# WeeFav/Visual-Odometry-GPU

Measured on AMD Instinct MI355X. Metric: ORB detect+describe frames/sec (1241x376, 8 lvls), higher is better.
Workload: dtype u8; 1 GPU; KITTI-shaped 1241x376 u8, 8 levels s=1.2, 1000 features, FAST-9 t=20, NMS 3x3, Harris top-N, blur5 all levels, BRIEF-256; batch=1024 frames/step/GPU resident in HBM (stream A); distinct_resident_batches=2, fast_early_exit=True, pyramid_blur_fused=True, pyramid_top_rows_first=True, pipelined_batches=True

## Files before the change

### visual-odometry-gpu_amd/csrc/orbx_kernels.hip

```cpp
#include <hip/hip_runtime.h>

#include <cstdlib>

#include "orbx_internal.h"
#include "orbx_math.h"
#include "orbx_wave.h"

__constant__ __attribute__((aligned(16))) int8_t c_pattern[1024] = {
#include "pattern_31.inc"
};


typedef uint16_t __attribute__((aligned(1))) u16_unaligned;

__device__ __forceinline__ void decode_tile(const OrbxTileMap& tm, int nlevels, int& l, int& tx, int& ty) {
  const int t = blockIdx.x;
  l = 0;
#pragma unroll 1
  for (int i = 1; i < nlevels; i++)
    if (t >= tm.begin[i]) l = i;
  const int local = t - tm.begin[l];
  ty = local / tm.tiles_x[l];
  tx = local - ty * tm.tiles_x[l];
}
// ... 6 lines not shown
}

typedef uint32_t __attribute__((aligned(1))) u32_unaligned;
struct __attribute__((packed, aligned(1))) uint2_unaligned {
  uint32_t x, y;
  __device__ operator uint2() const { return make_uint2(x, y); }
};

template <int ROWS, bool WIN8>
__device__ __forceinline__ void pyr_rows(const uint8_t* __restrict__ src, int in_stride, int w0, int h0,
                                         const OrbxResizeTap* __restrict__ ytaps, int yb, int lh,
                                         const uint32_t (&ofs)[4], const uint32_t (&cc)[4],
                                         __amdgpu_buffer_rsrc_t rout, uint32_t voff_st, uint32_t vmask, int pitch) {
  constexpr int NW = WIN8 ? 2 : 4;
  uint32_t q0[ROWS][NW], q1[ROWS][NW];
  int b0[ROWS], b1[ROWS];
  uint32_t sel[4];
  uint32_t base = 0;
  if (WIN8) {
    base = min(ofs[0], (uint32_t)(w0 - 8));
#pragma unroll
    for (int k = 0; k < 4; k++) {
      const uint32_t sb = ofs[k] - base;
      sel[k] = 0x0c000c00u | ((sb + 1) << 16) | sb;
    }
  }
#pragma unroll
  for (int r = 0; r < ROWS; r++) {
    const int y = min(yb + r, lh - 1);
    const OrbxResizeTap ty_ = ytaps[y];
    const int sy0 = min(max(ty_.ofs, 0), h0 - 1), sy1 = min(max(ty_.ofs + 1, 0), h0 - 1);
    const uint8_t* S0 = src + (size_t)sy0 * in_stride;
    const uint8_t* S1 = src + (size_t)sy1 * in_stride;
    b0[r] = ty_.c0;
    b1[r] = ty_.c1;
    if (WIN8) {
      const uint2 a = *reinterpret_cast<const uint2_unaligned*>(S0 + base);
      const uint2 b = *reinterpret_cast<const uint2_unaligned*>(S1 + base);
      q0[r][0] = a.x;
      q0[r][1] = a.y;
      q1[r][0] = b.x;
      q1[r][1] = b.y;
    } else {
#pragma unroll
      for (int k = 0; k < 4; k++) {
        q0[r][k] = *reinterpret_cast<const u16_unaligned*>(S0 + ofs[k]);
        q1[r][k] = *reinterpret_cast<const u16_unaligned*>(S1 + ofs[k]);
      }
    }
  }
#pragma unroll
  for (int r = 0; r < ROWS; r++) {
    uint32_t out = 0;
    const uint32_t bs0 = ((uint32_t)b0[r] << 12) & 0xffffffu, bs1 = ((uint32_t)b1[r] << 12) & 0xffffffu;
#pragma unroll
    for (int k = 0; k < 4; k++) {
      uint32_t p0, p1;
      if (WIN8) {
        p0 = __builtin_amdgcn_perm(q0[r][1], q0[r][0], sel[k]);
        p1 = __builtin_amdgcn_perm(q1[r][1], q1[r][0], sel[k]);
      } else {
        p0 = __builtin_amdgcn_perm(q0[r][k], q0[r][k], 0x0c010c00u);
        p1 = __builtin_amdgcn_perm(q1[r][k], q1[r][k], 0x0c010c00u);
      }
      const us2_t cw = __builtin_bit_cast(us2_t, cc[k]);
      const uint32_t r0 = __builtin_amdgcn_udot2(__builtin_bit_cast(us2_t, p0), cw, 0u, false);
      const uint32_t r1 = __builtin_amdgcn_udot2(__builtin_bit_cast(us2_t, p1), cw, 0u, false);
      const uint32_t t0 = (uint32_t)(((u64)(r0 & 0xfffff0u) * (u64)bs0) >> 32);
      const uint32_t t1 = (uint32_t)(((u64)(r1 & 0xfffff0u) * (u64)bs1) >> 32);
      out |= ((t0 + t1 + 2u) >> 2) << (8 * k);
    }
    const int y = yb + r;
    if (y < lh) __builtin_amdgcn_raw_buffer_store_b32(out & vmask, rout, voff_st, y * pitch, 0);
  }
}

__global__ __launch_bounds__(256) void k_pyramid2(const OrbxTileDesc* __restrict__ tiles, int n_tiles, int frame_bytes, int w0,
                                                  int h0, const uint8_t* __restrict__ in, int in_stride,
                                                  size_t in_frame_stride, const OrbxResizeTap* __restrict__ taps,
                                                  uint8_t* __restrict__ pyr) {
  if ((int)blockIdx.x >= n_tiles) return;
  const OrbxTileDesc d = tiles[blockIdx.x];
  struct {
    int w, h, pitch, xtab_off, ytab_off, win8;
  } L = {d.w, d.h, d.pitch, d.u0, d.u1, d.u2};
  const int l = d.l, tx = d.tx, ty = d.ty;
  const int rpw = d.f;
  const int f = blockIdx.y;
  const int lane = threadIdx.x & 63;
  const int wave = __builtin_amdgcn_readfirstlane(threadIdx.x >> 6);
  const uint8_t* src = in + (size_t)f * in_frame_stride;
  const int x = tx * 256 + lane * 4;
  const int yb = (ty * 4 + wave) * rpw;
  if (yb >= L.h) return;
  const int pitch = L.pitch, w = L.w;
  const __amdgpu_buffer_rsrc_t rout =
      __builtin_amdgcn_make_buffer_rsrc(pyr + (size_t)f * frame_bytes + d.img_off, 0, pitch * L.h, 0x00020000);
  const uint32_t voff_st = x < pitch ? (uint32_t)x : 0xffffffffu;
  const int nvalid = w - x;
  const uint32_t vmask = nvalid >= 4 ? 0xffffffffu : nvalid <= 0 ? 0u : ((1u << (8 * nvalid)) - 1u);

  if (l == 0) {
#pragma unroll
    for (int r = 0; r < 8; r++) {
      const int y = yb + r;
      if (r < rpw && y < L.h) {
        const uint8_t* row = src + (size_t)y * in_stride;
        uint32_t v = 0;
        if (nvalid >= 4 || (nvalid > 0 && y + 1 < L.h)) {
          v = *reinterpret_cast<const u32_unaligned*>(row + x);
        } else if (nvalid > 0) {
          for (int k = 0; k < nvalid; k++) v |= (uint32_t)row[x + k] << (8 * k);
        }
        __builtin_amdgcn_raw_buffer_store_b32(v & vmask, rout, voff_st, y * pitch, 0);
      }
    }
    return;
  }

  uint32_t ofs[4] = {0, 0, 0, 0}, cc[4] = {0, 0, 0, 0};
  if (nvalid > 0) {
    const uint4* tp = reinterpret_cast<const uint4*>(taps + L.xtab_off + x);
    const uint4 t01 = tp[0], t23 = tp[1];
    ofs[0] = t01.x; ofs[1] = t01.z; ofs[2] = t23.x; ofs[3] = t23.z;
    cc[0] = t01.y; cc[1] = t01.w; cc[2] = t23.y; cc[3] = t23.w;
  }
  const OrbxResizeTap* ytaps = taps + L.ytab_off;
  if (L.win8) {
    if (rpw == 8)
      pyr_rows<8, true>(src, in_stride, w0, h0, ytaps, yb, L.h, ofs, cc, rout, voff_st, vmask, pitch);
    else
      pyr_rows<4, true>(src, in_stride, w0, h0, ytaps, yb, L.h, ofs, cc, rout, voff_st, vmask, pitch);
  } else {
    pyr_rows<4, false>(src, in_stride, w0, h0, ytaps, yb, L.h, ofs, cc, rout, voff_st, vmask, pitch);
  }
}

#define BLUR_SROWS (ORBX_BLUR_TH + 4)
#define BLUR_SPITCH 72

__device__ __forceinline__ void blur_load_tile(uint8_t* s_src, const uint8_t* img, const OrbxLevel& L, int x0,
                                               int y0) {
  uint32_t* s32 = reinterpret_cast<uint32_t*>(s_src);
  for (int i = threadIdx.x; i < BLUR_SROWS * (BLUR_SPITCH / 4); i += 256) {
    const int row = i / (BLUR_SPITCH / 4), c = i - row * (BLUR_SPITCH / 4);
    const int gy = reflect101(y0 - 2 + row, L.h);
    const int gx = x0 - 4 + 4 * c;
    uint32_t v = 0;
    if (gx >= 0 && gx + 4 <= L.pitch) v = *reinterpret_cast<const uint32_t*>(img + (size_t)gy * L.pitch + gx);
    s32[i] = v;
  }
  __syncthreads();
  if (threadIdx.x < BLUR_SROWS) {
    uint8_t* row = s_src + threadIdx.x * BLUR_SPITCH;
    if (x0 == 0) {
      row[3] = row[5];
      row[2] = row[6];
    }
    const int rem = L.w - x0;
    if (rem <= ORBX_BLUR_TW + 1) {
#pragma unroll
      for (int k = 0; k < 2; k++) {
        const int x = L.w + k;
        const int col = x - x0 + 4;
        if (col < BLUR_SPITCH) row[col] = row[(2 * L.w - x - 2) - x0 + 4];
      }
    }
  }
  __syncthreads();
}

__global__ __launch_bounds__(256) void k_blur(OrbxPlan plan, OrbxTileMap tm, const uint8_t* __restrict__ src,
                                              uint8_t* __restrict__ dst, int first_level, int kind) {
  __shared__ __attribute__((aligned(16))) uint8_t s_src[BLUR_SROWS * BLUR_SPITCH];
  __shared__ __attribute__((aligned(16))) uint16_t s_h[BLUR_SROWS * ORBX_BLUR_TW];
  int l, tx, ty;
  decode_tile(tm, plan.nlevels, l, tx, ty);
  const OrbxLevel& L = plan.L[l];
  const int f = blockIdx.y;
  const uint8_t* img = src + (size_t)f * plan.frame_bytes + L.img_off;
  uint8_t* out = dst + (size_t)f * plan.frame_bytes + L.img_off;
  const int x0 = tx * ORBX_BLUR_TW, y0 = ty * ORBX_BLUR_TH;
  const int c4 = (threadIdx.x & 15) * 4, r = threadIdx.x >> 4;
  const int gy = y0 + r, gx = x0 + c4;

  if (l < first_level) {
    if (gy < L.h && gx < L.pitch)
      *reinterpret_cast<uint32_t*>(out + (size_t)gy * L.pitch + gx) =
          *reinterpret_cast<const uint32_t*>(img + (size_t)gy * L.pitch + gx);
    return;
  }
  blur_load_tile(s_src, img, L, x0, y0);

  uint32_t packed = 0;
  if (kind == 0) {
    for (int i = threadIdx.x; i < BLUR_SROWS * ORBX_BLUR_TW; i += 256) {
      const int row = i >> 6, c = i & 63;
      const uint8_t* p = s_src + row * BLUR_SPITCH + c + 2;
      s_h[i] = (uint16_t)(p[0] + 4 * p[1] + 6 * p[2] + 4 * p[3] + p[4]);
    }
    __syncthreads();
#pragma unroll
    for (int k = 0; k < 4; k++) {
      const uint16_t* h = s_h + r * ORBX_BLUR_TW + c4 + k;
      const uint32_t S = h[0] + 4u * h[ORBX_BLUR_TW] + 6u * h[2 * ORBX_BLUR_TW] + 4u * h[3 * ORBX_BLUR_TW] +
                         h[4 * ORBX_BLUR_TW];
      const uint32_t v = (S + 127u + ((S >> 8) & 1u)) >> 8;
      if (gx + k < L.w) packed |= v << (8 * k);
    }
  } else {
    const int kw[25] = {1, 4, 7, 4, 1, 4, 16, 26, 16, 4, 7, 26, 41, 26, 7, 4, 16, 26, 16, 4, 1, 4, 7, 4, 1};
#pragma unroll
    for (int k = 0; k < 4; k++) {
      uint32_t S = 0;
#pragma unroll
      for (int i = 0; i < 5; i++)
#pragma unroll
        for (int j = 0; j < 5; j++) S += (uint32_t)kw[i * 5 + j] * s_src[(r + i) * BLUR_SPITCH + c4 + k + 2 + j];
      const uint32_t v = (2u * S + 273u) / 546u;
      if (gx + k < L.w) packed |= v << (8 * k);
    }
  }
  if (gy < L.h && gx < L.pitch) *reinterpret_cast<uint32_t*>(out + (size_t)gy * L.pitch + gx) = packed;
}



__global__ __launch_bounds__(256) void k_compact(OrbxPlan plan, const u64* __restrict__ mask,
                                                 orbx_keypoint* __restrict__ cand,
                                                 int32_t* __restrict__ cand_count,
                                                 int32_t* __restrict__ cand_total, int need_total) {
  __shared__ int s_wsum[4];
  const int l = blockIdx.x, f = blockIdx.y;
  const OrbxLevel& L = plan.L[l];
  const u64* m = mask + (size_t)f * plan.mask_words + L.mask_off;
  orbx_keypoint* out = cand + (size_t)f * plan.cand_total + L.cand_off;
  const int nwords = L.h * L.mask_wpr;
  const int tid = threadIdx.x, lane = tid & 63, wave = tid >> 6;
  int base = 0;
  for (int w0 = 0; w0 < nwords; w0 += 256) {
    const int i = w0 + tid;
    u64 v = i < nwords ? m[i] : 0ull;
    const int c = __popcll(v);
    const int incl = wave_scan_incl(c);
    if (lane == 63) s_wsum[wave] = incl;
    __syncthreads();
    int woff = 0, tot = 0;
#pragma unroll
    for (int k = 0; k < 4; k++) {
      const int s = s_wsum[k];
      if (k < wave) woff += s;
      tot += s;
    }
    int pos = base + woff + incl - c;
    if (c && pos < L.cap) {
      const int y = i / L.mask_wpr, xw = i - y * L.mask_wpr;
      while (v && pos < L.cap) {
        const int b = __ffsll((long long)v) - 1;
        v &= v - 1;
        orbx_keypoint kp;
        kp.x = orbx_mask_x(L, xw, b);
        kp.y = y;
        out[pos++] = kp;
      }
    }
    base += tot;
    __syncthreads();
    if (!need_total && base >= L.cap) break;
  }
  if (tid == 0) {
    cand_total[f * plan.nlevels + l] = base;
    cand_count[f * plan.nlevels + l] = base < L.cap ? base : L.cap;
  }
}

__device__ __forceinline__ float harris_at(const uint8_t* img, int w, int h, int pitch, int x, int y,
                                           const float* __restrict__ g, int K, float kk) {
  const int r = K / 2;
  float a = 0.f, b = 0.f, c = 0.f;
  for (int i = 0; i < K; i++) {
    const int yy = reflect101(y - r + i, h);
    const uint8_t* r0 = img + (size_t)reflect101(yy - 1, h) * pitch;
    const uint8_t* r1 = img + (size_t)yy * pitch;
    const uint8_t* r2 = img + (size_t)reflect101(yy + 1, h) * pitch;
    for (int j = 0; j < K; j++) {
      const int xx = reflect101(x - r + j, w);
      const int xl = reflect101(xx - 1, w), xr = reflect101(xx + 1, w);
      const int p00 = r0[xl], p01 = r0[xx], p02 = r0[xr];
      const int p10 = r1[xl], p12 = r1[xr];
      const int p20 = r2[xl], p21 = r2[xx], p22 = r2[xr];
      const float gx = (float)((p02 + 2 * p12 + p22) - (p00 + 2 * p10 + p20));
      const float gy = (float)((p20 + 2 * p21 + p22) - (p00 + 2 * p01 + p02));
      const float wgt = g[i * K + j];
      a = __fadd_rn(a, __fmul_rn(__fmul_rn(gx, gx), wgt));
      c = __fadd_rn(c, __fmul_rn(__fmul_rn(gy, gy), wgt));
      b = __fadd_rn(b, __fmul_rn(__fmul_rn(gx, gy), wgt));
    }
  }
  const float det = __fsub_rn(__fmul_rn(a, c), __fmul_rn(b, b));
  const float trace = __fadd_rn(a, c);
  return __fsub_rn(det, __fmul_rn(__fmul_rn(kk, trace), trace));
}

template <int K>
__device__ __forceinline__ float harris_fast(const uint8_t* img, int w, int h, int pitch, int x, int y,
                                             const float* __restrict__ g, float kk) {
  constexpr int r = K / 2, P = K + 2;
  static_assert(P <= 9, "the third dword of a row supplies pixel 8 only");
  const int xs = x - r - 1;
  const int a0 = xs & ~3, off = xs - a0;
  const uint32_t sel_l = xs < 0 ? 0x03020102u : 0x03020100u;
  const uint32_t sel_r = xs + P - 1 >= w ? 0x0c0c0c06u : 0x0c0c0c00u;
  uint32_t raw[P][3];
#pragma unroll
  for (int i = 0; i < P; i++) {
    int yy = y - r - 1 + i;
    if (i == 0) yy = yy < 0 ? 1 : yy;
    if (i == P - 1) yy = yy >= h ? h - 2 : yy;
    const int o = yy * pitch + a0;
    raw[i][0] = *reinterpret_cast<const uint32_t*>(img + max(o, 0));
    raw[i][1] = *reinterpret_cast<const uint32_t*>(img + (o + 4));
    raw[i][2] = *reinterpret_cast<const uint32_t*>(img + (o + 8));
  }
  auto cvt_row = [&](int i, float (&out)[P]) {
    uint32_t q[3] = {__builtin_amdgcn_alignbyte(raw[i][1], raw[i][0], off),
                     __builtin_amdgcn_alignbyte(raw[i][2], raw[i][1], off), raw[i][2] >> (8 * off)};
    q[2] = __builtin_amdgcn_perm(q[1], q[2], sel_r);
    q[0] = __builtin_amdgcn_perm(q[0], q[0], sel_l);
#pragma unroll
    for (int j = 0; j < P; j++) out[j] = (float)((q[j >> 2] >> (8 * (j & 3))) & 0xffu);
  };
  auto hsum = [&](const float (&pr)[P], float (&out)[K]) {
#pragma unroll
    for (int j = 0; j < K; j++) out[j] = pr[j] + 2.0f * pr[j + 1] + pr[j + 2];
  };
  float pr[3][P], hs[3][K];
  cvt_row(0, pr[0]);
  cvt_row(1, pr[1]);
  hsum(pr[0], hs[0]);
  hsum(pr[1], hs[1]);
  float a = 0.f, b = 0.f, c = 0.f;
#pragma unroll
  for (int i = 0; i < K; i++) {
    float(&p0)[P] = pr[i % 3];
    float(&p1)[P] = pr[(i + 1) % 3];
    float(&p2)[P] = pr[(i + 2) % 3];
    cvt_row(i + 2, p2);
    hsum(p2, hs[(i + 2) % 3]);
    float vs[P];
#pragma unroll
    for (int j = 0; j < P; j++) vs[j] = p0[j] + 2.0f * p1[j] + p2[j];
#pragma unroll
    for (int j = 0; j < K; j++) {
      const float gx = vs[j + 2] - vs[j];
      const float gy = hs[(i + 2) % 3][j] - hs[i % 3][j];
      const float wgt = g[i * K + j];
      a = __fadd_rn(a, __fmul_rn(__fmul_rn(gx, gx), wgt));
      c = __fadd_rn(c, __fmul_rn(__fmul_rn(gy, gy), wgt));
      b = __fadd_rn(b, __fmul_rn(__fmul_rn(gx, gy), wgt));
    }
  }
  const float det = __fsub_rn(__fmul_rn(a, c), __fmul_rn(b, b));
  const float trace = __fadd_rn(a, c);
  return __fsub_rn(det, __fmul_rn(__fmul_rn(kk, trace), trace));
}

__device__ __forceinline__ bool harris_fast_ok(int w, int h, int x, int y, int K) {
  const int m = K / 2 + 1;
  return x >= m - 1 && y >= m - 1 && x <= w - m && y <= h - m && w >= 4 && h >= 4;
}

__device__ __forceinline__ float harris_any(const uint8_t* img, int w, int h, int pitch, int x, int y,
                                            const float* __restrict__ g, int K, float kk) {
  if (harris_fast_ok(w, h, x, y, K)) {
    if (K == 7) return harris_fast<7>(img, w, h, pitch, x, y, g, kk);
    if (K == 5) return harris_fast<5>(img, w, h, pitch, x, y, g, kk);
    if (K == 3) return harris_fast<3>(img, w, h, pitch, x, y, g, kk);
  }
  return harris_at(img, w, h, pitch, x, y, g, K, kk);
}

template <int K, int RPL, int G>
__device__ __forceinline__ float harris_row_group(const uint8_t* img, int pitch, int x, int y,
                                                  const float* __restrict__ g, float kk, int sub) {
  constexpr int r = K / 2, P = K + 2, NR = RPL + 2;
  constexpr int NL = (K + RPL - 1) / RPL;
  const int row0 = (sub < NL ? sub : NL - 1) * RPL;
  const int xs = x - r - 1;
  const int a0 = xs & ~3, off = xs - a0;
  float p[NR][P];
#pragma unroll
  for (int i = 0; i < NR; i++) {
    const int pr = min(row0 + i, P - 1);
    const uint32_t* row = reinterpret_cast<const uint32_t*>(img + (size_t)(y - r - 1 + pr) * pitch + a0);
    const uint32_t d0 = row[0], d1 = row[1], d2 = row[2];
    const uint32_t q[3] = {__builtin_amdgcn_alignbyte(d1, d0, off), __builtin_amdgcn_alignbyte(d2, d1, off),
                           d2 >> (8 * off)};
#pragma unroll
    for (int j = 0; j < P; j++) p[i][j] = (float)((q[j >> 2] >> (8 * (j & 3))) & 0xffu);
  }
  float hs[NR][K];
#pragma unroll
  for (int i = 0; i < NR; i++)
#pragma unroll
    for (int j = 0; j < K; j++) hs[i][j] = p[i][j] + 2.0f * p[i][j + 1] + p[i][j + 2];
  float pa[RPL][K], pb[RPL][K], pc[RPL][K];
#pragma unroll
  for (int w = 0; w < RPL; w++) {
    float vs[P];
#pragma unroll
    for (int j = 0; j < P; j++) vs[j] = p[w][j] + 2.0f * p[w + 1][j] + p[w + 2][j];
    const int wr = min(row0 + w, K - 1);
#pragma unroll
    for (int j = 0; j < K; j++) {
      const float gx = vs[j + 2] - vs[j], gy = hs[w + 2][j] - hs[w][j];
      const float wgt = g[wr * K + j];
      pa[w][j] = __fmul_rn(__fmul_rn(gx, gx), wgt);
      pc[w][j] = __fmul_rn(__fmul_rn(gy, gy), wgt);
      pb[w][j] = __fmul_rn(__fmul_rn(gx, gy), wgt);
    }
  }
  float a = 0.f, b = 0.f, c = 0.f;
#pragma unroll
  for (int rr = 0; rr < NL; rr++) {
    if (sub == rr) {
#pragma unroll
      for (int w = 0; w < RPL; w++)
        if (rr * RPL + w < K) {
#pragma unroll
          for (int j = 0; j < K; j++) {
            a = __fadd_rn(a, pa[w][j]);
            c = __fadd_rn(c, pc[w][j]);
            b = __fadd_rn(b, pb[w][j]);
          }
        }
    }
    if (rr + 1 < NL) {
      const float an = __builtin_bit_cast(float, __builtin_amdgcn_update_dpp(0, __builtin_bit_cast(int, a), 0x111, 0xf, 0xf, true));
      const float bn = __builtin_bit_cast(float, __builtin_amdgcn_update_dpp(0, __builtin_bit_cast(int, b), 0x111, 0xf, 0xf, true));
      const float cn = __builtin_bit_cast(float, __builtin_amdgcn_update_dpp(0, __builtin_bit_cast(int, c), 0x111, 0xf, 0xf, true));
      if (sub == rr + 1) {
        a = an;
        b = bn;
        c = cn;
      }
    }
  }
  const float det = __fsub_rn(__fmul_rn(a, c), __fmul_rn(b, b));
  const float trace = __fadd_rn(a, c);
  return __fsub_rn(det, __fmul_rn(__fmul_rn(kk, trace), trace));
}

template <int RPL, int G>
__device__ __forceinline__ float harris_group(const uint8_t* img, int w, int h, int pitch, int x, int y,
                                              const float* __restrict__ g, int K, float kk, int sub, bool active,
                                              bool& writer) {
  const int m = K / 2 + 1;
  const bool fast = (K == 7 || K == 5 || K == 3) && x >= m && y >= m && x < w - m && y < h - m;
  float res = 0.f;
  writer = false;
  const bool any_fast = __any(active && fast);
  if (any_fast) {
    const int xx = (active && fast) ? x : m, yy = (active && fast) ? y : m;
    float v = 0.f;
    int last = 0;
    if (K == 7) {
      v = harris_row_group<7, RPL, G>(img, pitch, xx, yy, g, kk, sub);
      last = (7 + RPL - 1) / RPL - 1;
    } else if (K == 5) {
      v = harris_row_group<5, RPL, G>(img, pitch, xx, yy, g, kk, sub);
      last = (5 + RPL - 1) / RPL - 1;
    } else {
      v = harris_row_group<3, RPL, G>(img, pitch, xx, yy, g, kk, sub);
      last = (3 + RPL - 1) / RPL - 1;
    }
    if (active && fast && sub == last) {
      res = v;
      writer = true;
    }
  }
  if (active && !fast && sub == 0) {
    res = harris_at(img, w, h, pitch, x, y, g, K, kk);
    writer = true;
  }
  return res;
}

__global__ __launch_bounds__(256) void k_harris2_flat(const uint8_t* __restrict__ img, int w, int h, int pitch,
                                                      const orbx_keypoint* __restrict__ kps, int nkp,
                                                      const float* __restrict__ gauss, int K, float kk,
                                                      float* __restrict__ resp) {
  constexpr int G = 8, RPL = 1;
  const int j = blockIdx.x * 32 + (threadIdx.x >> 3), sub = threadIdx.x & 7;
  const bool active = j < nkp;
  orbx_keypoint kp = {4, 4};
  if (active) kp = kps[j];
  bool writer;
  const float v = harris_group<RPL, G>(img, w, h, pitch, kp.x, kp.y, gauss, K, kk, sub, active, writer);
  if (writer) resp[j] = v;
}


#define LVL_THREADS 512
#define LVL_WAVES (LVL_THREADS / 64)
#define LVL_Q 16
#define LVL_RUN 64
#define LVL_MAX_SLOTS 4096

__host__ __device__ inline int lvl_slots(const OrbxPlan& plan, int nl) {
  int s = 0;
  for (int l = 0; l < nl; l++) s += (plan.L[l].cap + LVL_RUN - 1) & ~(LVL_RUN - 1);
  return s;
}

__device__ __forceinline__ u64 shfl_xor_u64(u64 v, int m) {
  const int lo = __shfl_xor((int)(uint32_t)v, m), hi = __shfl_xor((int)(uint32_t)(v >> 32), m);
  return ((u64)(uint32_t)hi << 32) | (uint32_t)lo;
}

__device__ __forceinline__ u64 wave_sort_desc(u64 k, int lane) {
#pragma unroll
  for (int b = 2; b <= 64; b <<= 1)
#pragma unroll
    for (int j = b >> 1; j > 0; j >>= 1) {
      const u64 o = shfl_xor_u64(k, j);
      const bool keep_max = ((lane & j) == 0) == ((lane & b) == 0);
      k = keep_max ? (o > k ? o : k) : (o < k ? o : k);
    }
  return k;
}

__device__ __forceinline__ int lvl_of_run(const int* s_runs, int l0, int l1, int& r) {
  int l = l0;
  while (l < l1 - 1) {
    const int c = __builtin_amdgcn_readfirstlane(s_runs[l]);
    if (r < c) break;
    r -= c;
    l++;
  }
  return l;
}

template <int KF>
__global__ __launch_bounds__(LVL_THREADS) __attribute__((amdgpu_waves_per_eu(4, 8))) void k_level_select(
    OrbxPlan plan, int lpg, int mode, const u64* __restrict__ mask, const uint8_t* __restrict__ pyr,
    const float* __restrict__ gauss, int K, float kk, orbx_keypoint* __restrict__ sel_lkp,
    float* __restrict__ sel_resp, int32_t* __restrict__ sel_count, uint32_t* __restrict__ need) {
  extern __shared__ __attribute__((aligned(16))) unsigned char s_dyn[];
  __shared__ int s_n[ORBX_MAX_LEVELS];
  __shared__ int s_runs[ORBX_MAX_LEVELS];
  const int f = blockIdx.x, nl = plan.nlevels;
  const int l0 = blockIdx.y * lpg, l1 = min(l0 + lpg, nl);
  const int nslots = lvl_slots(plan, nl);
  u64* s_key = reinterpret_cast<u64*>(s_dyn);
  uint32_t* s_kp = reinterpret_cast<uint32_t*>(s_dyn + 8 * (size_t)nslots);
  float* s_r = reinterpret_cast<float*>(s_dyn + 12 * (size_t)nslots);
  const int tid = threadIdx.x, lane = tid & 63;
  const int wave = __builtin_amdgcn_readfirstlane(tid >> 6);
  const size_t fo = (size_t)f * plan.out_cap;

  for (int l = l0 + wave; l < l1; l += LVL_WAVES) {
    const OrbxLevel& L = plan.L[l];
    const int cap = L.cap, slot = lvl_slots(plan, l);
    const u64* m = mask + (size_t)f * plan.mask_words + L.mask_off;
    const int nwords = L.h * L.mask_wpr;
    int base = 0, last = -1;
    for (int w0 = 0; w0 < nwords && base < cap; w0 += 64 * LVL_Q) {
      u64 v[LVL_Q];
#pragma unroll
      for (int q = 0; q < LVL_Q; q++) {
        const int i = w0 + 64 * q + lane;
        v[q] = i < nwords ? m[i] : 0ull;
      }
#pragma unroll
      for (int q = 0; q < LVL_Q; q++) {
        const int c = __popcll(v[q]);
        const int incl = wave_scan_incl(c);
        int pos = base + incl - c;
        if (c && pos < cap) {
          const int i = w0 + 64 * q + lane;
          const int y = i / L.mask_wpr, xw = i - y * L.mask_wpr;
          u64 w = v[q];
          while (w && pos < cap) {
            const int b = __ffsll((long long)w) - 1;
            w &= w - 1;
            const int x = orbx_mask_x(L, xw, b);
            if (mode == ORBX_SELECT_ROWMAJOR) {
              orbx_keypoint kp;
              kp.x = x;
              kp.y = y;
              sel_lkp[fo + L.out_off + pos] = kp;
              sel_resp[fo + L.out_off + pos] = 0.0f;
            } else {
              s_kp[slot + pos] = ((uint32_t)y << 16) | (uint32_t)x;
            }
            if (pos == cap - 1) last = y;
            pos++;
          }
        }
        base += __builtin_amdgcn_readlane(incl, 63);
      }
    }
    const int n = base < cap ? base : cap;
    const int keep = n < L.quota ? n : L.quota;
    const int runs = (n + LVL_RUN - 1) / LVL_RUN;
    const u64 found = __ballot(last >= 0);
    const int last_row = found ? __builtin_amdgcn_readlane(last, __ffsll((long long)found) - 1) : L.h - 1;
    if (lane == 0) {
      s_n[l] = n;
      s_runs[l] = runs;
      sel_count[f * nl + l] = keep;
      if (need && cap > 0) atomicMax(&need[l], (uint32_t)last_row + 1u);
    }
  }
  if (mode == ORBX_SELECT_ROWMAJOR) return;
  __syncthreads();

  int nruns = 0;
  for (int l = l0; l < l1; l++) nruns += s_runs[l];
  nruns = __builtin_amdgcn_readfirstlane(nruns);
  const uint8_t* img_f = pyr + (size_t)f * plan.frame_bytes;
  if (KF > 0) {
    for (int t = wave; t < nruns; t += LVL_WAVES) {
      int r = t;
      const int l = lvl_of_run(s_runs, l0, l1, r);
      const OrbxLevel& L = plan.L[l];
      const int slot = lvl_slots(plan, l), i = LVL_RUN * r + lane;
      const bool live = i < __builtin_amdgcn_readfirstlane(s_n[l]);
      const uint32_t p = live ? s_kp[slot + i] : 0u;
      const int x = (int)(p & 0xffffu), y = (int)(p >> 16);
      const bool fast = live && harris_fast_ok(L.w, L.h, x, y, KF);
      if (fast) s_r[slot + i] = harris_fast<KF>(img_f + L.img_off, L.w, L.h, L.pitch, x, y, gauss, kk);
    }
  }
  for (int t = wave; t < nruns; t += LVL_WAVES) {
    int r = t;
    const int l = lvl_of_run(s_runs, l0, l1, r);
    const OrbxLevel& L = plan.L[l];
    const int slot = lvl_slots(plan, l), i = LVL_RUN * r + lane;
    u64 key = 0ull;
    if (i < __builtin_amdgcn_readfirstlane(s_n[l])) {
      const uint32_t p = s_kp[slot + i];
      const int x = (int)(p & 0xffffu), y = (int)(p >> 16);
      const bool fast = KF > 0 && harris_fast_ok(L.w, L.h, x, y, KF);
      float resp;
      if (fast) {
        resp = s_r[slot + i];
      } else {
        resp = harris_at(img_f + L.img_off, L.w, L.h, L.pitch, x, y, gauss, K, kk);
        s_r[slot + i] = resp;
      }
      uint32_t u = orbx_f2u(resp);
      if (u == 0x80000000u) u = 0u;
      u ^= (u >> 31) ? 0xffffffffu : 0x80000000u;
      key = ((u64)u << 32) | (uint32_t)~(uint32_t)i;
    }
    s_key[slot + i] = wave_sort_desc(key, lane);
  }
  __syncthreads();
  for (int t = wave; t < nruns; t += LVL_WAVES) {
    int r = t;
    const int l = lvl_of_run(s_runs, l0, l1, r);
    const int slot = lvl_slots(plan, l);
    const int runs = __builtin_amdgcn_readfirstlane(s_runs[l]);
    const u64 k = s_key[slot + LVL_RUN * r + lane];
    int rank = lane;
    for (int o = 0; o < runs; o++) {
      if (o == r) continue;
      const u64* run = s_key + slot + LVL_RUN * o;
      int c = 0;
#pragma unroll
      for (int step = LVL_RUN / 2; step > 0; step >>= 1) c += run[c + step - 1] > k ? step : 0;
      c += run[c] > k;
      rank += c;
    }
    const int n = __builtin_amdgcn_readfirstlane(s_n[l]);
    const int keep = n < plan.L[l].quota ? n : plan.L[l].quota;
    if (k != 0ull && rank < keep) {
      const int i = (int)~(uint32_t)k;
      const uint32_t p = s_kp[slot + i];
      orbx_keypoint kp;
      kp.x = (int)(p & 0xffffu);
      kp.y = (int)(p >> 16);
      const size_t so = fo + plan.L[l].out_off + rank;
      sel_lkp[so] = kp;
      sel_resp[so] = s_r[slot + i];
    }
  }
}

__global__ __launch_bounds__(256) void k_lvl_compact(OrbxPlan plan, const u64* __restrict__ mask,
                                                     uint32_t* __restrict__ cand, int32_t* __restrict__ ncand,
                                                     uint32_t* __restrict__ need) {
  __shared__ int s_wsum[4][4];
  const int l = blockIdx.x, f = blockIdx.y;
  const OrbxLevel& L = plan.L[l];
  const int cap = L.cap;
  const u64* m = mask + (size_t)f * plan.mask_words + L.mask_off;
  uint32_t* out = cand + (size_t)f * plan.cand_total + L.cand_off;
  const int nwords = L.h * L.mask_wpr;
  const int tid = threadIdx.x, lane = tid & 63, wave = tid >> 6;
  int base = 0;
  for (int w0 = 0; w0 < nwords && base < cap; w0 += 1024) {
    u64 v[4];
#pragma unroll
    for (int q = 0; q < 4; q++) {
      const int i = w0 + 256 * q + tid;
      v[q] = i < nwords ? m[i] : 0ull;
    }
    int incl[4], c[4];
#pragma unroll
    for (int q = 0; q < 4; q++) {
      c[q] = __popcll(v[q]);
      incl[q] = wave_scan_incl(c[q]);
      if (lane == 63) s_wsum[q][wave] = incl[q];
    }
    __syncthreads();
#pragma unroll
    for (int q = 0; q < 4; q++) {
      int woff = 0, tot = 0;
#pragma unroll
      for (int k = 0; k < 4; k++) {
        const int sv = s_wsum[q][k];
        if (k < wave) woff += sv;
        tot += sv;
      }
      int pos = base + woff + incl[q] - c[q];
      if (c[q] && pos < cap) {
        const int i = w0 + 256 * q + tid;
        const int y = i / L.mask_wpr, xw = i - y * L.mask_wpr;
        u64 w = v[q];
        while (w && pos < cap) {
          const int b = __ffsll((long long)w) - 1;
          w &= w - 1;
          out[pos++] = ((uint32_t)y << 16) | (uint32_t)orbx_mask_x(L, xw, b);
        }
      }
      base += tot;
    }
    __syncthreads();
  }
  if (tid == 0) ncand[f * plan.nlevels + l] = base < cap ? base : cap;
  if (need && tid == 0 && cap > 0) atomicMax(&need[l], base >= cap ? (out[cap - 1] >> 16) + 1u : (uint32_t)L.h);
}

__global__ __launch_bounds__(256) __attribute__((amdgpu_waves_per_eu(4, 8))) void k_lvl_harris(
    OrbxPlan plan, const uint8_t* __restrict__ pyr, const float* __restrict__ gauss, int K, float kk,
    const uint32_t* __restrict__ cand, const int32_t* __restrict__ ncand, float* __restrict__ resp) {
  const int l = blockIdx.y, f = blockIdx.z;
  const OrbxLevel& L = plan.L[l];
  const int n = ncand[f * plan.nlevels + l];
  const int i = blockIdx.x * 256 + threadIdx.x;
  if ((int)blockIdx.x * 256 >= n) return;
  if (i >= n) return;
  const size_t o = (size_t)f * plan.cand_total + L.cand_off + i;
  const uint32_t p = cand[o];
  const uint8_t* img = pyr + (size_t)f * plan.frame_bytes + L.img_off;
  resp[o] = harris_any(img, L.w, L.h, L.pitch, (int)(p & 0xffffu), (int)(p >> 16), gauss, K, kk);
}

#define RANK_SLICE 64
__global__ __launch_bounds__(256) void k_lvl_rank(OrbxPlan plan, const uint32_t* __restrict__ cand,
                                                  const int32_t* __restrict__ ncand, const float* __restrict__ resp,
                                                  orbx_keypoint* __restrict__ sel_lkp, float* __restrict__ sel_resp,
                                                  int32_t* __restrict__ sel_count) {
  extern __shared__ __attribute__((aligned(16))) unsigned char s_dyn[];
  __shared__ int s_part[4][RANK_SLICE];
  u64* s_key = reinterpret_cast<u64*>(s_dyn);
  const int l = blockIdx.y, f = blockIdx.z;
  const OrbxLevel& L = plan.L[l];
  const int n = ncand[f * plan.nlevels + l];
  const int keep = n < L.quota ? n : L.quota;
  const int tid = threadIdx.x;
  if (blockIdx.x == 0 && tid == 0) sel_count[f * plan.nlevels + l] = keep;
  const int first = blockIdx.x * RANK_SLICE;
  if (first >= n) return;
  const size_t co = (size_t)f * plan.cand_total + L.cand_off;
  const int n8 = (n + 7) & ~7;
  for (int i = tid; i < n8; i += 256) {
    u64 key = 0ull;
    if (i < n) {
      uint32_t u = orbx_f2u(resp[co + i]);
      if (u == 0x80000000u) u = 0u;
      u ^= (u >> 31) ? 0xffffffffu : 0x80000000u;
      key = ((u64)u << 32) | (uint32_t)~(uint32_t)i;
    }
    s_key[i] = key;
  }
  __syncthreads();
  const int ci = tid & (RANK_SLICE - 1), part = tid >> 6;
  const int i = first + ci;
  const u64 ki = s_key[i < n8 ? i : 0];
  const int per = n8 / 4;
  int rank = 0;
  for (int j = part * per; j < (part + 1) * per; j += 2) {
    const ulonglong2 v = *reinterpret_cast<const ulonglong2*>(&s_key[j]);
    rank += v.x > ki;
    rank += v.y > ki;
  }
  s_part[part][ci] = rank;
  __syncthreads();
  if (part == 0 && i < n) {
    rank = s_part[0][ci] + s_part[1][ci] + s_part[2][ci] + s_part[3][ci];
    if (rank < keep) {
      const uint32_t p = cand[co + i];
      const size_t so = (size_t)f * plan.out_cap + L.out_off;
      orbx_keypoint kp;
      kp.x = (int)(p & 0xffffu);
      kp.y = (int)(p >> 16);
      sel_lkp[so + rank] = kp;
      sel_resp[so + rank] = resp[co + i];
    }
  }
}

__global__ __launch_bounds__(256) void k_select_flat(const float* __restrict__ resp, int n, int keep,
                                                     int32_t* __restrict__ idx) {
  const int m = n < keep ? n : keep;
  for (int i = blockIdx.x * 256 + threadIdx.x; i < n; i += gridDim.x * 256) {
    const float ri = resp[i];
    int rank = 0;
    for (int j = 0; j < n; j++) {
      const float rj = resp[j];
      rank += (rj > ri) || (rj == ri && j < i);
    }
    if (rank < m) idx[rank] = i;
  }
}

#define DESC_R 20
#define DESC_ROWS (2 * DESC_R + 1)
#define DESC_PITCH 48
#define DESC_HP 40
#define DESC_BROWS (DESC_ROWS - 4)

struct DescLds {
  union {
    uint32_t patch[DESC_ROWS * DESC_PITCH / 4];
    uint16_t box[DESC_BROWS * DESC_HP];
  };
  uint16_t hs[DESC_ROWS * DESC_HP];
};

__device__ __forceinline__ u64 hsum5x4(uint32_t d0, uint32_t d1) {
  const u64 acc = (u64)__builtin_amdgcn_perm(d1, d1, 0x0c010c00u) |
                  ((u64)__builtin_amdgcn_perm(d1, d1, 0x0c030c02u) << 32);
  return __builtin_amdgcn_qsad_pk_u16_u8((u64)d0 | ((u64)d1 << 32), 0u, acc);
}

struct DescJob {
  const uint8_t* img;
  int w, h, pitch;
  int x, y;
  bool valid;
};

__device__ __forceinline__ void describe_wave(const DescJob& jb, DescLds& lds, int patch_size,
                                              bool use_given_angle, float given_angle, bool do_brief,
                                              float& angle_out, u64 desc_out[4]) {
  const int lane = lane_id();
  const uint8_t* s_patch = reinterpret_cast<const uint8_t*>(lds.patch);
  const int px0 = jb.x - DESC_R, py0 = jb.y - DESC_R;
  const int ax0 = px0 & ~3;
  const int off = px0 - ax0;
  if (jb.valid) {
    int row = lane / (DESC_PITCH / 4), c = lane - row * (DESC_PITCH / 4);
#pragma unroll
    for (int k = 0; k < (DESC_ROWS * (DESC_PITCH / 4) + 63) / 64; k++) {
      const int i = lane + 64 * k;
      if (i < DESC_ROWS * (DESC_PITCH / 4)) {
        const int gy = py0 + row, gx = ax0 + 4 * c;
        uint32_t v = 0;
        if ((unsigned)gy < (unsigned)jb.h && (unsigned)gx < (unsigned)jb.pitch)
          v = *reinterpret_cast<const uint32_t*>(jb.img + (uint32_t)(gy * jb.pitch + gx));
        lds.patch[i] = v;
      }
      row += 5;
      c += 4;
      if (c >= DESC_PITCH / 4) {
        c -= DESC_PITCH / 4;
        row += 1;
      }
    }
  }
  __syncthreads();
  float angle = 0.0f;
  if (jb.valid) {
    if (use_given_angle) {
      angle = given_angle;
    } else {
      const int pr = patch_size / 2, P = 2 * pr + 1;
      if (!(jb.x - pr < 0 || jb.x + pr >= jb.w || jb.y - pr < 0 || jb.y + pr >= jb.h)) {
        const int grp_shift = P <= 32 ? 5 : 6;
        const int col = lane & ((1 << grp_shift) - 1), grp = lane >> grp_shift, ngrp = 64 >> grp_shift;
        int colsum = 0, m01 = 0;
        if (col < P) {
          const uint8_t* pc = s_patch + (DESC_R - pr) * DESC_PITCH + (col - pr + DESC_R + off);
          for (int rr = grp; rr < P; rr += ngrp) {
            const int I = pc[rr * DESC_PITCH];
            colsum += I;
            m01 += (rr - pr) * I;
          }
        }
        int m10 = (col - pr) * colsum;
        m10 = wave_sum(m10);
        m01 = wave_sum(m01);
        angle = orbx_atan2f((float)m01, (float)m10);
      }
    }
  }
  angle_out = angle;
  if (!do_brief) return;

  if (jb.valid) {
    int r = lane / 10, g = lane - r * 10;
#pragma unroll
    for (int k = 0; k < (DESC_ROWS * 10 + 63) / 64; k++) {
      if (lane + 64 * k < DESC_ROWS * 10) {
        const uint32_t d0 = lds.patch[r * (DESC_PITCH / 4) + g], d1 = lds.patch[r * (DESC_PITCH / 4) + g + 1];
        *reinterpret_cast<u64*>(&lds.hs[r * DESC_HP + 4 * g]) = hsum5x4(d0, d1);
      }
      r += 6;
      g += 4;
      if (g >= 10) {
        g -= 10;
        r += 1;
      }
    }
  }
  __syncthreads();
  if (jb.valid) {
    int r = lane / 10, g = lane - r * 10;
#pragma unroll
    for (int k = 0; k < (DESC_BROWS * 10 + 63) / 64; k++) {
      if (lane + 64 * k < DESC_BROWS * 10) {
        const uint2* hp = reinterpret_cast<const uint2*>(&lds.hs[r * DESC_HP + 4 * g]);
        uint2 acc = hp[0];
#pragma unroll
        for (int q = 1; q < 5; q++) {
          const uint2 v = hp[q * (DESC_HP / 4)];
          acc.x = pk_add(acc.x, v.x);
          acc.y = pk_add(acc.y, v.y);
        }
        *reinterpret_cast<uint2*>(&lds.box[r * DESC_HP + 4 * g]) = acc;
      }
      r += 6;
      g += 4;
      if (g >= 10) {
        g -= 10;
        r += 1;
      }
    }
  }
  __syncthreads();

  const float c = orbx_cosf(angle), s = orbx_sinf(angle);
#pragma unroll 1
  for (int k = 0; k < 4; k++) {
    bool bit = false;
    if (jb.valid) {
      const int i = k * 64 + lane;
      const int32_t pk = reinterpret_cast<const int32_t*>(c_pattern)[i];
      const float x1 = (float)(int8_t)(pk & 0xff), y1 = (float)(int8_t)((pk >> 8) & 0xff);
      const float x2 = (float)(int8_t)((pk >> 16) & 0xff), y2 = (float)(int8_t)((pk >> 24) & 0xff);
      int dx1 = orbx_lroundf(__fsub_rn(__fmul_rn(c, x1), __fmul_rn(s, y1)));
      int dy1 = orbx_lroundf(__fadd_rn(__fmul_rn(s, x1), __fmul_rn(c, y1)));
      int dx2 = orbx_lroundf(__fsub_rn(__fmul_rn(c, x2), __fmul_rn(s, y2)));
      int dy2 = orbx_lroundf(__fadd_rn(__fmul_rn(s, x2), __fmul_rn(c, y2)));
      const int cx1 = jb.x + dx1, cy1 = jb.y + dy1, cx2 = jb.x + dx2, cy2 = jb.y + dy2;
      const bool skip = cx1 < 2 || cy1 < 2 || cx1 > jb.w - 1 || cy1 > jb.h - 1 || cx2 < 2 || cy2 < 2 ||
                        cx2 > jb.w - 1 || cy2 > jb.h - 1;
      if (!skip) {
        dx1 = min(max(dx1, -18), 18);
        dy1 = min(max(dy1, -18), 18);
        dx2 = min(max(dx2, -18), 18);
        dy2 = min(max(dy2, -18), 18);
        const int s1 = lds.box[(dy1 + 18) * DESC_HP + dx1 + 18 + off];
        const int s2 = lds.box[(dy2 + 18) * DESC_HP + dx2 + 18 + off];
        bit = s1 < s2;
      }
    }
    desc_out[k] = __ballot(bit);
  }
}



#define DESC_NLD ((DESC_ROWS * (DESC_PITCH / 4) + 63) / 64)

struct DescClip {
  int rlo, rhi, clo, chi;
};
__device__ __forceinline__ DescClip desc_clip(const DescJob& jb) {
  const int py0 = jb.y - DESC_R, ax0 = (jb.x - DESC_R) & ~3;
  return {max(-py0, 0), min(jb.h - 1 - py0, DESC_ROWS - 1), max(-ax0, 0), min(jb.pitch - 4 - ax0, DESC_PITCH - 4)};
}
enum { DESC_INSIDE = 0, DESC_TOP = 1, DESC_CLIPPED = 2 };
__device__ __forceinline__ int desc_kind(const DescJob& jb) {
  const int py0 = jb.y - DESC_R, ax0 = (jb.x - DESC_R) & ~3;
  const bool below = py0 + DESC_ROWS <= jb.h, cols = ax0 >= 0 && ax0 + DESC_PITCH <= jb.pitch;
  return below && cols ? (py0 >= 0 ? DESC_INSIDE : DESC_TOP) : DESC_CLIPPED;
}

template <int KIND>
__device__ __forceinline__ void desc_fetch_border(const DescJob& jb, uint32_t base, const int (&rowk)[DESC_NLD],
                                                  const int (&c3)[3], uint32_t (&regs)[DESC_NLD]) {
  const DescClip cl = desc_clip(jb);
  int cb[3];
#pragma unroll
  for (int m = 0; m < 3; m++) cb[m] = KIND == DESC_TOP ? 4 * c3[m] : min(max(4 * c3[m], cl.clo), cl.chi);
#pragma unroll
  for (int k = 0; k < DESC_NLD; k++) {
    const int r = KIND == DESC_TOP ? max(rowk[k], cl.rlo) : min(max(rowk[k], cl.rlo), cl.rhi);
    regs[k] = *reinterpret_cast<const uint32_t*>(
        jb.img + (base + (__umul24((uint32_t)r, (uint32_t)jb.pitch) + (uint32_t)cb[k % 3])));
  }
}

struct DescLds2 {
  uint32_t patch[DESC_ROWS * DESC_PITCH / 4];
  uint16_t hs[DESC_ROWS * DESC_HP];
};

template <class L>
__device__ __forceinline__ void desc_store_patch(L& lds, int lane, const uint32_t (&regs)[DESC_NLD]) {
#pragma unroll
  for (int k = 0; k < DESC_NLD; k++)
    if (lane + 64 * k < DESC_ROWS * (DESC_PITCH / 4)) lds.patch[lane + 64 * k] = regs[k];
}

template <class L>
__device__ __forceinline__ void desc_zero_outside(L& lds, int lane, const DescClip& cl) {
  constexpr int RD = DESC_PITCH / 4;
  for (int i = lane; i < RD * cl.rlo; i += 64) lds.patch[i] = 0;
  for (int i = RD * (cl.rhi + 1) + lane; i < RD * DESC_ROWS; i += 64) lds.patch[i] = 0;
  if (lane < DESC_ROWS) {
    for (int c = 0; c < cl.clo / 4; c++) lds.patch[lane * RD + c] = 0;
    for (int c = cl.chi / 4 + 1; c < RD; c++) lds.patch[lane * RD + c] = 0;
  }
}

#define DESC_TAG 0x8000u
template <class L>
__device__ __forceinline__ void desc_tag_outside(L& lds, int lane, const DescJob& jb, int off) {
  constexpr int RD = DESC_HP / 2;
  const int rlo = min(max(DESC_R - jb.y, 0), DESC_BROWS), rhi = max(min(jb.h + 17 - jb.y, DESC_BROWS - 1), -1);
  const int jlo = min(max(DESC_R + off - jb.x, 0), DESC_HP), jhi = max(min(jb.w + 17 + off - jb.x, DESC_HP - 1), -1);
  uint32_t* t32 = reinterpret_cast<uint32_t*>(lds.hs);
  for (int i = lane; i < RD * rlo; i += 64) t32[i] = DESC_TAG * 0x10001u;
// ... 579 lines not shown
```

Measured before the change: 607,500 frames/s.

## Pack Harris Sobel sums into 16-bit pairs and raise select kernel occupancy

```diff
diff --git a/visual-odometry-gpu_amd/csrc/orbx_kernels.hip b/visual-odometry-gpu_amd/csrc/orbx_kernels.hip
--- a/visual-odometry-gpu_amd/csrc/orbx_kernels.hip
+++ b/visual-odometry-gpu_amd/csrc/orbx_kernels.hip
@@ -332,62 +332,85 @@
   return __fsub_rn(det, __fmul_rn(__fmul_rn(kk, trace), trace));
 }
 
+#define HARRIS_AHEAD 2
 template <int K>
 __device__ __forceinline__ float harris_fast(const uint8_t* img, int w, int h, int pitch, int x, int y,
                                              const float* __restrict__ g, float kk) {
   constexpr int r = K / 2, P = K + 2;
+  constexpr int NE = (P + 1) / 2, NH = (K + 1) / 2;
   static_assert(P <= 9, "the third dword of a row supplies pixel 8 only");
   const int xs = x - r - 1;
   const int a0 = xs & ~3, off = xs - a0;
-  const uint32_t sel_l = xs < 0 ? 0x03020102u : 0x03020100u;
-  const uint32_t sel_r = xs + P - 1 >= w ? 0x0c0c0c06u : 0x0c0c0c00u;
+  constexpr int dr = P - 1, sr = P - 3;
+  constexpr uint32_t id = 0x03020100u;
+  constexpr uint32_t rfl = (id & ~(0xffu << (8 * (dr & 3)))) | ((uint32_t)(4 + (sr & 3)) << (8 * (dr & 3)));
+  const uint32_t sel_l = xs < 0 ? 0x03020102u : id;
+  const uint32_t sel_r = xs + P - 1 >= w ? rfl : id;
   uint32_t raw[P][3];
-#pragma unroll
-  for (int i = 0; i < P; i++) {
+  auto fetch = [&](int i) {
     int yy = y - r - 1 + i;
     if (i == 0) yy = yy < 0 ? 1 : yy;
     if (i == P - 1) yy = yy >= h ? h - 2 : yy;
     const int o = yy * pitch + a0;
-    raw[i][0] = *reinterpret_cast<const uint32_t*>(img + max(o, 0));
-    raw[i][1] = *reinterpret_cast<const uint32_t*>(img + (o + 4));
-    raw[i][2] = *reinterpret_cast<const uint32_t*>(img + (o + 8));
-  }
-  auto cvt_row = [&](int i, float (&out)[P]) {
+    const uint32_t o1 = (uint32_t)(o + 4);
+    raw[i][0] = *reinterpret_cast<const uint32_t*>(img + (uint32_t)max(o, 0));
+    raw[i][1] = *reinterpret_cast<const uint32_t*>(img + o1);
+    raw[i][2] = *reinterpret_cast<const uint32_t*>(img + o1 + 4);
+  };
+  auto pair = [&](const uint32_t (&q)[3], int pa, int pb) {
+    const uint32_t sel = 0x0c000c00u | (uint32_t)(pa & 3) | (pb < P ? (uint32_t)(4 + (pb & 3)) << 16 : 0x000c0000u);
+    return __builtin_amdgcn_perm(q[pb < P ? pb >> 2 : 0], q[pa >> 2], sel);
+  };
+  auto unpack = [&](int i, uint32_t (&e)[NE], uint32_t (&hs)[NH]) {
     uint32_t q[3] = {__builtin_amdgcn_alignbyte(raw[i][1], raw[i][0], off),
                      __builtin_amdgcn_alignbyte(raw[i][2], raw[i][1], off), raw[i][2] >> (8 * off)};
-    q[2] = __builtin_amdgcn_perm(q[1], q[2], sel_r);
+    q[dr >> 2] = __builtin_amdgcn_perm(q[sr >> 2], q[dr >> 2], sel_r);
     q[0] = __builtin_amdgcn_perm(q[0], q[0], sel_l);
 #pragma unroll
-    for (int j = 0; j < P; j++) out[j] = (float)((q[j >> 2] >> (8 * (j & 3))) & 0xffu);
+    for (int k = 0; k < NE; k++) e[k] = pair(q, 2 * k, 2 * k + 1);
+#pragma unroll
+    for (int k = 0; k < NH; k++) {
+      const uint32_t o = pair(q, 2 * k + 1, 2 * k + 2);
+      hs[k] = pk_add(pk_add(e[k], o), pk_add(o, e[k + 1]));
+    }
   };
-  auto hsum = [&](const float (&pr)[P], float (&out)[K]) {
-#pragma unroll
-    for (int j = 0; j < K; j++) out[j] = pr[j] + 2.0f * pr[j + 1] + pr[j + 2];
-  };
-  float pr[3][P], hs[3][K];
-  cvt_row(0, pr[0]);
-  cvt_row(1, pr[1]);
-  hsum(pr[0], hs[0]);
-  hsum(pr[1], hs[1]);
+#pragma unroll
+  for (int i = 0; i < HARRIS_AHEAD && i < P; i++) fetch(i);
+  uint32_t e0[NE], e1[NE], t[NE], hs[3][NH];
+  if (HARRIS_AHEAD < P) fetch(HARRIS_AHEAD);
+  unpack(0, e0, hs[0]);
+  if (HARRIS_AHEAD + 1 < P) fetch(HARRIS_AHEAD + 1);
+  unpack(1, e1, hs[1]);
+#pragma unroll
+  for (int k = 0; k < NE; k++) t[k] = pk_add(e0[k], e1[k]);
   float a = 0.f, b = 0.f, c = 0.f;
 #pragma unroll
   for (int i = 0; i < K; i++) {
-    float(&p0)[P] = pr[i % 3];
-    float(&p1)[P] = pr[(i + 1) % 3];
-    float(&p2)[P] = pr[(i + 2) % 3];
-    cvt_row(i + 2, p2);
-    hsum(p2, hs[(i + 2) % 3]);
-    float vs[P];
-#pragma unroll
-    for (int j = 0; j < P; j++) vs[j] = p0[j] + 2.0f * p1[j] + p2[j];
-#pragma unroll
-    for (int j = 0; j < K; j++) {
-      const float gx = vs[j + 2] - vs[j];
-      const float gy = hs[(i + 2) % 3][j] - hs[i % 3][j];
-      const float wgt = g[i * K + j];
-      a = __fadd_rn(a, __fmul_rn(__fmul_rn(gx, gx), wgt));
-      c = __fadd_rn(c, __fmul_rn(__fmul_rn(gy, gy), wgt));
-      b = __fadd_rn(b, __fmul_rn(__fmul_rn(gx, gy), wgt));
+    if (i + 2 + HARRIS_AHEAD < P) fetch(i + 2 + HARRIS_AHEAD);
+    uint32_t e2[NE], vs[NE];
+    unpack(i + 2, e2, hs[(i + 2) % 3]);
+#pragma unroll
+    for (int k = 0; k < NE; k++) {
+      const uint32_t t2 = pk_add(e1[k], e2[k]);
+      vs[k] = pk_add(t[k], t2);
+      t[k] = t2;
+      e1[k] = e2[k];
+    }
+#pragma unroll
+    for (int k = 0; k < NH; k++) {
+      const uint32_t gx2 = pk_sub(vs[k + 1], vs[k]);
+      const uint32_t gy2 = pk_sub(hs[(i + 2) % 3][k], hs[i % 3][k]);
+#pragma unroll
+      for (int s = 0; s < 2; s++) {
+        const int j = 2 * k + s;
+        if (j >= K) break;
+        const float gx = s ? (float)((int32_t)gx2 >> 16) : (float)(int16_t)gx2;
+        const float gy = s ? (float)((int32_t)gy2 >> 16) : (float)(int16_t)gy2;
+        const float wgt = g[i * K + j];
+        a = __fadd_rn(a, __fmul_rn(__fmul_rn(gx, gx), wgt));
+        c = __fadd_rn(c, __fmul_rn(__fmul_rn(gy, gy), wgt));
+        b = __fadd_rn(b, __fmul_rn(__fmul_rn(gx, gy), wgt));
+      }
     }
   }
   const float det = __fsub_rn(__fmul_rn(a, c), __fmul_rn(b, b));
@@ -571,8 +594,14 @@
   return l;
 }
 
+__device__ __forceinline__ int lane_reread() {
+  uint32_t z = 0;
+  asm volatile("" : "+v"(z));
+  return (int)__builtin_amdgcn_mbcnt_hi(~0u, __builtin_amdgcn_mbcnt_lo(~0u, z));
+}
+
 template <int KF>
-__global__ __launch_bounds__(LVL_THREADS) __attribute__((amdgpu_waves_per_eu(4, 8))) void k_level_select(
+__global__ __launch_bounds__(LVL_THREADS) __attribute__((amdgpu_waves_per_eu(6, 8))) void k_level_select(
     OrbxPlan plan, int lpg, int mode, const u64* __restrict__ mask, const uint8_t* __restrict__ pyr,
     const float* __restrict__ gauss, int K, float kk, orbx_keypoint* __restrict__ sel_lkp,
     float* __restrict__ sel_resp, int32_t* __restrict__ sel_count, uint32_t* __restrict__ need) {
@@ -596,20 +625,20 @@
     const int nwords = L.h * L.mask_wpr;
     int base = 0, last = -1;
     for (int w0 = 0; w0 < nwords && base < cap; w0 += 64 * LVL_Q) {
+      const int i0 = w0 + LVL_Q * lane;
       u64 v[LVL_Q];
+      int tot = 0;
 #pragma unroll
       for (int q = 0; q < LVL_Q; q++) {
-        const int i = w0 + 64 * q + lane;
-        v[q] = i < nwords ? m[i] : 0ull;
-      }
-#pragma unroll
-      for (int q = 0; q < LVL_Q; q++) {
-        const int c = __popcll(v[q]);
-        const int incl = wave_scan_incl(c);
-        int pos = base + incl - c;
-        if (c && pos < cap) {
-          const int i = w0 + 64 * q + lane;
-          const int y = i / L.mask_wpr, xw = i - y * L.mask_wpr;
+        v[q] = i0 + q < nwords ? m[i0 + q] : 0ull;
+        tot += __popcll(v[q]);
+      }
+      const int incl = wave_scan_incl(tot);
+      int pos = base + incl - tot;
+      if (tot && pos < cap) {
+        int y = i0 / L.mask_wpr, xw = i0 - y * L.mask_wpr;
+#pragma unroll
+        for (int q = 0; q < LVL_Q; q++) {
           u64 w = v[q];
           while (w && pos < cap) {
             const int b = __ffsll((long long)w) - 1;
@@ -627,9 +656,13 @@
             if (pos == cap - 1) last = y;
             pos++;
           }
+          if (++xw == L.mask_wpr) {
+            xw = 0;
+            y++;
+          }
         }
-        base += __builtin_amdgcn_readlane(incl, 63);
-      }
+      }
+      base += __builtin_amdgcn_readlane(incl, 63);
     }
     const int n = base < cap ? base : cap;
     const int keep = n < L.quota ? n : L.quota;
@@ -650,24 +683,28 @@
   for (int l = l0; l < l1; l++) nruns += s_runs[l];
   nruns = __builtin_amdgcn_readfirstlane(nruns);
   const uint8_t* img_f = pyr + (size_t)f * plan.frame_bytes;
-  if (KF > 0) {
+  if constexpr (KF > 0) {
     for (int t = wave; t < nruns; t += LVL_WAVES) {
       int r = t;
       const int l = lvl_of_run(s_runs, l0, l1, r);
       const OrbxLevel& L = plan.L[l];
-      const int slot = lvl_slots(plan, l), i = LVL_RUN * r + lane;
+      const int slot = lvl_slots(plan, l), i = LVL_RUN * r + lane_reread();
       const bool live = i < __builtin_amdgcn_readfirstlane(s_n[l]);
       const uint32_t p = live ? s_kp[slot + i] : 0u;
       const int x = (int)(p & 0xffffu), y = (int)(p >> 16);
       const bool fast = live && harris_fast_ok(L.w, L.h, x, y, KF);
-      if (fast) s_r[slot + i] = harris_fast<KF>(img_f + L.img_off, L.w, L.h, L.pitch, x, y, gauss, kk);
+      if (fast) {
+        const float resp = harris_fast<KF>(img_f + L.img_off, L.w, L.h, L.pitch, x, y, gauss, kk);
+        s_r[slot + LVL_RUN * r + lane_reread()] = resp;
+      }
     }
   }
   for (int t = wave; t < nruns; t += LVL_WAVES) {
     int r = t;
     const int l = lvl_of_run(s_runs, l0, l1, r);
     const OrbxLevel& L = plan.L[l];
-    const int slot = lvl_slots(plan, l), i = LVL_RUN * r + lane;
+    const int ln = lane_reread();
+    const int slot = lvl_slots(plan, l), i = LVL_RUN * r + ln;
     u64 key = 0ull;
     if (i < __builtin_amdgcn_readfirstlane(s_n[l])) {
       const uint32_t p = s_kp[slot + i];
@@ -685,7 +722,7 @@
       u ^= (u >> 31) ? 0xffffffffu : 0x80000000u;
       key = ((u64)u << 32) | (uint32_t)~(uint32_t)i;
     }
-    s_key[slot + i] = wave_sort_desc(key, lane);
+    s_key[slot + i] = wave_sort_desc(key, ln);
   }
   __syncthreads();
   for (int t = wave; t < nruns; t += LVL_WAVES) {
@@ -693,8 +730,9 @@
     const int l = lvl_of_run(s_runs, l0, l1, r);
     const int slot = lvl_slots(plan, l);
     const int runs = __builtin_amdgcn_readfirstlane(s_runs[l]);
-    const u64 k = s_key[slot + LVL_RUN * r + lane];
-    int rank = lane;
+    const int ln = lane_reread();
+    const u64 k = s_key[slot + LVL_RUN * r + ln];
+    int rank = ln;
     for (int o = 0; o < runs; o++) {
       if (o == r) continue;
       const u64* run = s_key + slot + LVL_RUN * o;
@@ -774,7 +812,7 @@
   if (need && tid == 0 && cap > 0) atomicMax(&need[l], base >= cap ? (out[cap - 1] >> 16) + 1u : (uint32_t)L.h);
 }
 
-__global__ __launch_bounds__(256) __attribute__((amdgpu_waves_per_eu(4, 8))) void k_lvl_harris(
+__global__ __launch_bounds__(256) __attribute__((amdgpu_waves_per_eu(6, 8))) void k_lvl_harris(
     OrbxPlan plan, const uint8_t* __restrict__ pyr, const float* __restrict__ gauss, int K, float kk,
     const uint32_t* __restrict__ cand, const int32_t* __restrict__ ncand, float* __restrict__ resp) {
   const int l = blockIdx.y, f = blockIdx.z;
```

Measured after the change: 633,200 frames/s (median of 6 runs). 1.04x the previous value.
